# westi024/RadTxfr

Measured on AMD Instinct MI355X. Metric: wavenumber*layer points/s (32-layer TUD, 500-6000 cm^-1 @ 0.001 cm^-1), higher is better.
Workload: dtype f32; 1 GPU; C3: 32-layer TUD (tau,Lu,Ld) StandardAtmosphere rows 1-32, 500-6000 cm^-1 @ 0.001 cm^-1; n_wavenumbers=5500000, n_layers=32, n_lines=100000, n_angles=30, line_table=synthetic HITRAN-format H2O+CO2, seed 20261005, parallelism=wavenumber-sharded x1, pipelines_per_gpu=3

## Files before the change

### include/radtxfr_hip.h

```cpp
#ifndef RADTXFR_HIP_H
#define RADTXFR_HIP_H

#include <stdint.h>

#ifdef __cplusplus
extern "C" {
#endif

#define RTX_VERSION 100

typedef struct rtx_grid {
  double xmin;
  double xmax;
  double step;
  int64_t n_total;
  int64_t offset;
  int64_t n;
} rtx_grid;

int rtx_version(void);
const char* rtx_last_error(void);
int rtx_device_info(char* name_h, int len, int* n_cu_h);

typedef struct rtx_lines rtx_lines;
// ... 33 lines not shown
                         const double* T_h, const double* T_win_h, const double* p_atm_h, const double* qratio_h,
                         const double* weight_h, const double* mass_h, double dil_air, double dil_self,
                         double omega_wing, double omega_wing_hw, double intensity_threshold, double scale,
                         int profile, void* stream);

int rtx_line_prep_axis(rtx_prep* prep, const rtx_lines* lines, const double* X_h, int64_t nx, int n_layers,
                       const double* T_h, const double* p_atm_h, const double* qratio_h, const double* weight_h,
                       const double* mass_h, double dil_air, double dil_self, double omega_wing, double omega_wing_hw,
                       double intensity_threshold, double scale, int profile, void* stream);

#define RTX_MAX_DILUENTS 8
int rtx_line_prep_mix(rtx_prep* prep, const rtx_lines* lines, const rtx_grid* grid, int n_layers, const double* T_h,
                      const double* p_atm_h, const double* qratio_h, const double* weight_h, const double* mass_h,
                      int n_dil, const int32_t* dil_h, const double* frac_h, double omega_wing, double omega_wing_hw,
                      double intensity_threshold, double scale, int profile, void* stream);
int rtx_line_prep_axis_mix(rtx_prep* prep, const rtx_lines* lines, const double* X_h, int64_t nx, int n_layers,
                           const double* T_h, const double* p_atm_h, const double* qratio_h, const double* weight_h,
                           const double* mass_h, int n_dil, const int32_t* dil_h, const double* frac_h, double omega_wing,
                           double omega_wing_hw, double intensity_threshold, double scale, int profile, void* stream);

int rtx_voigt_tile_points(void);
int rtx_voigt_sum(const rtx_prep* prep, const rtx_grid* grid, int n_layers, float* out_f32,
                  double* out_f64, int64_t ld, void* stream);
int rtx_voigt_sum_axis(const rtx_prep* prep, int n_layers, float* out_f32, double* out_f64, int64_t ld, void* stream);

int rtx_line_prep_dt(rtx_prep* prep, const rtx_lines* lines, const rtx_grid* grid, int n_layers, const double* T_h,
                     const double* p_atm_h, const double* qratio_h, const double* weight_h, const double* mass_h,
                     const double* dlnsw_h, double dil_air, double dil_self, double omega_wing, double omega_wing_hw,
                     double intensity_threshold, double scale, void* stream);
int rtx_voigt_sum_dt(const rtx_prep* prep, const rtx_grid* grid, int n_layers, float* out_f32, double* out_f64,
                     int64_t ld, void* stream);

int rtx_planck(const rtx_grid* grid, const double* X, int64_t nx, const double* T, int64_t nT,
               int wavelength, double* out, void* stream);

int rtx_brightness_temperature(const double* X, int64_t nx, const double* L, int64_t m,
                               int wavelength, double bad_value, double* T_out, void* stream);
int rtx_bt2l(const double* X, int64_t nx, const double* T, int64_t m, int wavelength,
             double bad_value, double* L_out, void* stream);

int rtx_tud(const float* OD, int64_t ld, const rtx_grid* grid, int n_layers, const double* T_h,
            int n_alt, const uint8_t* mask_h, int n_mu, const double* mu_h, int n_down,
            int n_angle, int return_od, float* tau, float* Lu, float* Ld, float* Ld_angles,
            int64_t ld_out, void* stream);
#define RTX_TUD_OD_NONNEG 1u
int rtx_tud_opts(const float* OD, int64_t ld, const rtx_grid* grid, int n_layers, const double* T_h,
// ... 210 lines not shown
```

### radtxfr_amd/_lib.py

```python
import ctypes as C
import os

_HERE = os.path.dirname(os.path.abspath(__file__))
LIB_PATH = os.environ.get("RADTXFR_LIB") or os.path.join(_HERE, "libradtxfr_hip.so")


class RtxGrid(C.Structure):
    _fields_ = [("xmin", C.c_double), ("xmax", C.c_double), ("step", C.c_double),
                ("n_total", C.c_int64), ("offset", C.c_int64), ("n", C.c_int64)]


_vp, _i64, _i32, _dbl = C.c_void_p, C.c_int64, C.c_int, C.c_double
_pd = C.POINTER(C.c_double)
_gp = C.POINTER(RtxGrid)

PROTOTYPES = {
    "rtx_version": (_i32, []),
    "rtx_last_error": (C.c_char_p, []),
    "rtx_device_info": (_i32, [C.c_char_p, _i32, C.POINTER(_i32)]),
    "rtx_lines_create": (_i32, [_i64, _i32] + [_vp] * 10 + [_vp, C.POINTER(_vp)]),
    "rtx_lines_free": (_i32, [_vp]),
    "rtx_lines_count": (_i64, [_vp]),
    "rtx_prep_create": (_i32, [_vp, _i32, _i64, C.POINTER(_vp)]),
    "rtx_prep_free": (_i32, [_vp]),
    "rtx_line_prep": (_i32, [_vp, _vp, _gp, _i32, _vp, _vp, _vp, _vp, _vp, _dbl, _dbl, _dbl, _dbl, _dbl, _dbl, _vp]),
    "rtx_line_prep_profile": (_i32, [_vp, _vp, _gp, _i32, _vp, _vp, _vp, _vp, _vp, _dbl, _dbl, _dbl, _dbl, _dbl, _dbl, _i32, _vp]),
    "rtx_prep_split_bound": (_i64, [_vp]),
    "rtx_line_prep_window": (_i32, [_vp, _vp, _gp, _i32, _vp, _vp, _vp, _vp, _vp, _vp, _dbl, _dbl, _dbl, _dbl, _dbl, _dbl, _i32, _vp]),
    "rtx_line_prep_axis": (_i32, [_vp, _vp, _vp, _i64, _i32, _vp, _vp, _vp, _vp, _vp, _dbl, _dbl, _dbl, _dbl, _dbl, _dbl, _i32, _vp]),
    "rtx_voigt_sum": (_i32, [_vp, _gp, _i32, _vp, _vp, _i64, _vp]),
    "rtx_voigt_sum_axis": (_i32, [_vp, _i32, _vp, _vp, _i64, _vp]),
    "rtx_sdvoigt_sum": (_i32, [_vp, _gp, _i32, _vp, _vp, _i64, _vp]),
    "rtx_lines_set_sd": (_i32, [_vp, _vp, _vp]),
    "rtx_lines_set_deltap_self": (_i32, [_vp, _vp]),
    "rtx_lines_set_broadeners": (_i32, [_vp, _i32, _vp, _vp, _vp, _vp, _vp]),
    "rtx_line_prep_mix": (_i32, [_vp, _vp, _gp, _i32, _vp, _vp, _vp, _vp, _vp, _i32, _vp, _vp, _dbl, _dbl, _dbl, _dbl, _i32, _vp]),
    "rtx_line_prep_axis_mix": (_i32, [_vp, _vp, _vp, _i64, _i32, _vp, _vp, _vp, _vp, _vp, _i32, _vp, _vp, _dbl, _dbl, _dbl, _dbl,
                                       _i32, _vp]),
    "rtx_voigt_tile_points": (_i32, []),
    "rtx_planck": (_i32, [_gp, _vp, _i64, _vp, _i64, _i32, _vp, _vp]),
    "rtx_tud": (_i32, [_vp, _i64, _gp, _i32, _vp, _i32, _vp, _i32, _vp, _i32, _i32, _i32, _vp, _vp, _vp, _vp, _i64, _vp]),
    "rtx_tud_opts": (_i32, [_vp, _i64, _gp, _i32, _vp, _i32, _vp, _i32, _vp, _i32, _i32, _i32, _vp, _vp, _vp, _vp, _i64, _vp, C.c_uint]),
    "rtx_tud_jacobian": (_i32, [_vp, _vp, _vp, _i64, _dbl, _vp, _i32, _vp, _i64, _gp, _i32, _vp, _i32, _vp, _dbl, _i32, _i32,
                                 _i32, _vp, _i32, _i32, _vp, _i64, _vp]),
    "rtx_tud_vjp": (_i32, [_vp, _vp, _vp, _i64, _dbl, _vp, _i32, _vp, _i64, _gp, _i32, _vp, _i32, _vp, _dbl, _i32, _i32,
                            _i32, _vp, _i32, _i32, _vp, _vp, _vp, _i64, _i32, _vp, _vp]),
    "rtx_tud_vjp_max_vectors": (_i32, []),
    "rtx_line_prep_dt": (_i32, [_vp, _vp, _gp, _i32, _vp, _vp, _vp, _vp, _vp, _vp, _dbl, _dbl, _dbl, _dbl, _dbl, _dbl, _vp]),
    "rtx_voigt_sum_dt": (_i32, [_vp, _gp, _i32, _vp, _vp, _i64, _vp]),
    "rtx_tud_jacobian_dod": (_i32, [_vp, _vp, _i64, _vp, _i32, _vp, _i64, _gp, _i32, _vp, _i32, _vp, _dbl, _i32, _i32,
                                     _i32, _vp, _i32, _i32, _vp, _i64, _vp]),
    "rtx_tud_vjp_dod": (_i32, [_vp, _vp, _i64, _vp, _i32, _vp, _i64, _gp, _i32, _vp, _i32, _vp, _dbl, _i32, _i32,
                                _i32, _vp, _i32, _i32, _vp, _vp, _vp, _i64, _i32, _vp, _vp]),
# ... 113 lines not shown
```

### radtxfr_amd/csrc/rtx_voigt.hip

```cpp
#include <stdlib.h>
#include <string.h>

#include "rtx_common.h"

#include "rtx_voigt_math.h"

struct RangeArgs {
  const int* ic;
  const int* maxhw;
  const int2* win;
  long long n_lines;
  int n_tiles, tile, n_layers, n_steps;
  long long n;
  int2* ranges;
  SplitItem* items;
  int* n_items;
  long long items_cap;
};

#define RNG_G 16
__device__ __forceinline__ unsigned group_bits(unsigned long long b, int lane) { return (unsigned)(b >> (lane & 48)) & 0xffffu; }

template <bool STRICT>
__device__ __forceinline__ void bound_step(const int* __restrict__ ic, int& lo, int& hi, int v, int sub, int lane) {
// ... 124 lines not shown
    if (out_f32) RTX_HIP(hipMemset2DAsync(out_f32, ld * sizeof(float), 0, grid->n * sizeof(float), n_layers, st));
    if (out_f64) RTX_HIP(hipMemset2DAsync(out_f64, ld * sizeof(double), 0, grid->n * sizeof(double), n_layers, st));
    return 0;
  }
  return rtx_voigt_sum_scatter(P, grid, n_layers, out_f32, out_f64, ld, st, launch_tile_ranges, voigt_kernel_choice() == 0);
}

bool rtx_voigt_layers_ok(const rtx_prep* P) {
  return P && !P->axis && P->n_lines > 0 && voigt_kernel_choice() == 0 && !(P->split_bound > 0 && P->items.get());
}
int rtx_voigt_sum_layers(const rtx_prep* P, const rtx_grid* grid, int n_layers, float* out_f32, int64_t ld, void* stream,
                         const VoigtLayers& sel) {
  if (!rtx_voigt_layers_ok(P)) RTX_FAIL("internal: a layer subset on a prologue that cannot take one");
  if (rtx_check_grid(grid)) return 1;
  if (n_layers < 1 || n_layers != P->n_layers) RTX_FAIL("n_layers=%d does not match the last rtx_line_prep (%d)", n_layers, P->n_layers);
  if (!out_f32) RTX_FAIL("the output is NULL");
  if (ld < grid->n) RTX_FAIL("ld=%lld < n=%lld", (long long)ld, (long long)grid->n);
  if (sel.n_a < 0 || sel.n_y < sel.n_a || sel.n_y < 1 || sel.k_a < 0 || sel.k_a + sel.n_a > n_layers || sel.k_b < 0 ||
      sel.k_b + (sel.n_y - sel.n_a) > n_layers)
    RTX_FAIL("internal: layer subset outside [0,%d)", n_layers);
  if (grid->n == 0) return 0;
  return rtx_voigt_sum_scatter(P, grid, n_layers, out_f32, nullptr, ld, (hipStream_t)stream, launch_tile_ranges, 1, &sel);
}
```

### radtxfr_amd/csrc/rtx_voigt_scatter.hip

```cpp
#include "rtx_common.h"

#include "rtx_voigt_math.h"

#include "cheb8_64.inc"
#include "cheb16_tile.inc"
#include <vector>

#ifndef RTX_SC_ABLATE
#define RTX_SC_ABLATE 0
#endif
#ifndef RTX_SC_ASYM
#define RTX_SC_ASYM 1
#endif
#ifndef RTX_SC_OUTER
#define RTX_SC_OUTER 1
#endif
#ifndef RTX_SC_ROWS
#define RTX_SC_ROWS 16
#endif
#ifndef RTX_SC_NEAR
#define RTX_SC_NEAR 2
#endif
static_assert(RTX_SC_ROWS <= 31, "row masks are 32-bit");

// ... 300 lines not shown
#endif
#ifndef SC_EDGE_LIST
#define SC_EDGE_LIST 1
#endif
#ifndef SC_EDGE_CAP
#define SC_EDGE_CAP 32
#endif
#ifndef SC_EDGE_UNROLL
#define SC_EDGE_UNROLL 2
#endif
#ifndef RTX_SC_TILE_LEVEL
#define RTX_SC_TILE_LEVEL 1
#endif
#define RTX_SC_TILE_DIST 512
#ifndef RTX_SC_RED_REG
#define RTX_SC_RED_REG 1
#endif
#ifndef RTX_SC_MERGE
#define RTX_SC_MERGE 1
#endif
#ifndef RTX_SC_BAND_SPLIT
#define RTX_SC_BAND_SPLIT 1
#endif
#ifndef SC_ENT_CAP
#define SC_ENT_CAP (SC_EDGE_LIST ? 16 : 32)
#endif
template <bool SMALLY, bool PARTS = false>
__device__ __forceinline__ void nodal_tile(const ScArgs& a, const int b_or_tile, const int k, const int2 part_rng = make_int2(0, 0),
                                           float* __restrict__ part_out = nullptr, const unsigned done_rows = 0u) {
  constexpr int ROWS = RTX_SC_ROWS;
  constexpr int TILE = 64 * ROWS;
  __shared__ float s_acc[SC_NW][TILE];
  __shared__ float4 s_ent[SC_NW][SC_ENT_CAP][4];
  __shared__ float4 s_edge[SC_NW][SC_EDGE_LIST ? SC_EDGE_CAP : 1][2];
  __shared__ float s_nodsum[RTX_SC_ROWS][CHEB_N];
  static_assert((RTX_SC_ROWS * CHEB_N + TCHEB_N + 1) * 4 <= SC_ENT_CAP * 64, "row sums + tile sums fit in one wave's entry list");

  const int tile = part_out ? b_or_tile : xcd_tile(b_or_tile);
  if (tile >= a.n_tiles) return;
  const int wave = __builtin_amdgcn_readfirstlane((int)(threadIdx.x >> 6));
  const int lane = threadIdx.x & 63;
  const long long n = a.g.n;
  const int ia = tile * TILE;
  const int ib = (int)((long long)ia + TILE < n ? (long long)ia + TILE : n);
  const int nt = ib - ia;
  const LineRec* __restrict__ rec = a.rec + (size_t)k * (size_t)a.n_lines;
  const LineRec64* __restrict__ rec64 = a.rec64 + (size_t)k * (size_t)a.n_lines;
  const int2 rng = part_out ? part_rng : a.ranges[(size_t)k * a.n_tiles + tile];
  float* __restrict__ acc = s_acc[wave];
#pragma unroll
  for (int r = 0; r < ROWS; ++r) acc[r * 64 + lane] = 0.f;
  const float lanef = (float)lane;
  bool touched = false;
// ... 1 lines not shown
  long long t_prev = RTX_SC_STAMP ? (long long)clock64() : 0;
  const long long t_begin = t_prev;

  const int l = lane >> 3, j = lane & 7;
  float nod[ROWS];
#pragma unroll
  for (int r = 0; r < ROWS; ++r) nod[r] = 0.f;
  constexpr bool TILE_LEVEL = RTX_SC_TILE_LEVEL && ROWS == 16;
#ifndef RTX_SC_OFF_LDS
#define RTX_SC_OFF_LDS 0
#endif
#if !RTX_SC_OFF_LDS
  const float off_j = CHEB_OFF[j];
#endif
  if (lane < 8) {
    int lt = lane;
    if (SMALLY) asm volatile("" : "+v"(lt));
    s_nodsum[wave][lane] = CHEB_OFF[lt];
    if (TILE_LEVEL) s_nodsum[SC_NW + wave][lane] = TCHEB_OFF[lt];
  }
  float tnod_a = 0.f, tnod_b = 0.f;
  int n_tile_members = 0;
  int n_ent = 0;
  float4(*__restrict__ ent)[4] = s_ent[wave];
  auto below = [](unsigned long long m) -> int {
    return (int)__builtin_amdgcn_mbcnt_hi((unsigned)(m >> 32), __builtin_amdgcn_mbcnt_lo((unsigned)m, 0u));
  };
  auto pull = [](int src_lane, float v) -> float {
    return __int_as_float(__builtin_amdgcn_ds_bpermute(src_lane << 2, __float_as_int(v)));
  };

  static_assert(ROWS <= 16, "an entry packs its row masks as 16-bit halves");
  auto drain = [&]() {
    for (int e = 0; e < n_ent; ++e) {
      const float4 e0 = ent[e][0], e1 = ent[e][1], e2 = ent[e][2], e3 = ent[e][3];
      LineRec q;
      q.a = e0.x; q.c = e0.y; q.b1 = e0.z; q.b0 = e0.w;
      q.Ay = e1.x; q.Ay0 = e1.y; q.y = e1.z; q.A = e1.w;
      const float u0 = e2.x + lanef, ulo = e2.y, uhi = e2.z, zw_f = e2.w;
      const unsigned w0 = (unsigned)__builtin_amdgcn_readfirstlane(__float_as_int(e3.x));
      const unsigned w1 = (unsigned)__builtin_amdgcn_readfirstlane(__float_as_int(e3.y));
      unsigned m_pp = w0 & 0xffffu, m_ed = w0 >> 16, m_bd = w1 & 0xffffu, m_cut = w1 >> 16;
      if (!PARTS) {
        m_pp &= ~done_rows; m_ed &= ~done_rows;
      }
      auto slot = [&]() -> int { return __builtin_amdgcn_readfirstlane(__float_as_int(ent[e][3].z)); };
      STAMP(3);
      if (RTX_SC_ABLATE & 4) m_pp = m_ed = 0u;
      while (m_pp) {
        const int r = __builtin_ctz(m_pp);
        m_pp &= m_pp - 1u;
        float* p = acc + r * 64 + lane;
        float x0, n0, d0;
        farwing(u0 + (float)(64 * r), q, x0, n0, d0);
        p[0] = fmaf(n0, d0, p[0]);
      }
      while (m_ed) {
        const int r = __builtin_ctz(m_ed);
        m_ed &= m_ed - 1u;
        float* p = acc + r * 64 + lane;
        const float u = u0 + (float)(64 * r);
        float x0, n0, d0;
        farwing(u, q, x0, n0, d0);
        n0 = (u >= ulo && u < uhi) ? n0 : 0.f;
        p[0] = fmaf(n0, d0, p[0]);
      }
// ... 15 lines not shown
              p[0] = fmaf(num, rden, p[0]);
            }
          } else {
            for (; r < r_end; ++r) {
              float* p = acc + r * 64 + lane;
              float num, rden;
              band_row<0, false, 0>(a, rec64, slot, q, u0 + (float)(64 * r), ia + 64 * r + lane, zw_f, ulo, uhi, false, num, rden, touched);
              p[0] = fmaf(num, rden, p[0]);
            }
          }
        }
        while (m_cut) {
          const int r = __builtin_ctz(m_cut);
          m_cut &= m_cut - 1u;
          float* p = acc + r * 64 + lane;
          float num, rden;
          band_row<SMALLY ? 2 : 0>(a, rec64, slot, q, u0 + (float)(64 * r), ia + 64 * r + lane, zw_f, ulo, uhi, small_y, num, rden, touched);
          p[0] = fmaf(num, rden, p[0]);
        }
      }
      STAMP(5);
    }
    n_ent = 0;
  };

  int n_edge = 0;
  float4(*__restrict__ edg)[2] = s_edge[wave];
  auto edge_one = [&](const float4& E0, const float4& E1, int pk) {
    const int r = (pk >> 7) & 31, t = pk & 127;
    const bool right = (pk >> 12) & 1;
    float* p = acc + r * 64 + lane;
    const float u = E1.z + lanef;
    const float x = fmaf(u, E0.x, E0.y);
    const float xx = x * x;
    float num = fmaf(xx, E1.x, E1.y);
    const float rden = __builtin_amdgcn_rcpf(fmaf(xx + E0.z, xx, E0.w));
    const bool inside = (lane >= t) != right;
    num = inside ? num : 0.f;
    p[0] = fmaf(num, rden, p[0]);
  };
  auto drain_edges = [&]() {
    for (int e = 0; e < n_edge; e += SC_EDGE_UNROLL) {
      float4 E0[SC_EDGE_UNROLL], E1[SC_EDGE_UNROLL];
      int pk[SC_EDGE_UNROLL];
#pragma unroll
      for (int q = 0; q < SC_EDGE_UNROLL; ++q) {
        const int eq = e + q < n_edge ? e + q : e;
        E0[q] = edg[eq][0];
        E1[q] = edg[eq][1];
      }
#pragma unroll
      for (int q = 0; q < SC_EDGE_UNROLL; ++q) pk[q] = __builtin_amdgcn_readfirstlane(__float_as_int(E1[q].w));
#pragma unroll
      for (int q = 0; q < SC_EDGE_UNROLL; ++q)
        if (e + q < n_edge) edge_one(E0[q], E1[q], pk[q]);
    }
    n_edge = 0;
  };

  for (int base = rng.x + wave; base < rng.y; base += 64 * SC_NW) {
    const int slot = base + SC_NW * lane;
    const bool valid = slot < rng.y;
    const float4* __restrict__ pr = reinterpret_cast<const float4*>(rec + (valid ? slot : rng.y - 1));
    const float4 f0 = pr[0];
    const float4 f1 = pr[1];
    const float4 f2 = pr[2];
    const int qi0 = __float_as_int(f2.x), qlo = __float_as_int(f2.y), qhi = __float_as_int(f2.z), qzw = __float_as_int(f2.w);
    const bool reach = valid && qhi > ia && qlo < ib;
    const RowGeom g = row_geom(qi0, qlo, qhi, qzw, ia, nt);
    auto bits = [](int lo, int hi) -> unsigned {
      return hi > lo ? (((1u << hi) - 1u) & ~((1u << lo) - 1u)) : 0u;
    };
    const unsigned m_reach = reach ? bits(g.r_lo, g.r_hi) : 0u;
    const unsigned m_in = reach ? bits(g.c0, g.c1) : 0u;
    const unsigned m_near = bits(g.n0 > 0 ? g.n0 : 0, (g.n1 < ROWS - 1 ? g.n1 : ROWS - 1) + 1);
    const unsigned m_band = bits(g.z0, g.z1 + 1);
    const unsigned m_far = (RTX_SC_ABLATE & 2) ? 0u : (m_in & ~m_near);
    const unsigned m_bd = m_reach & m_band;
    const unsigned m_pp = m_in & m_near & ~m_band;
    const unsigned m_ed = (RTX_SC_ABLATE & 16) ? 0u : (m_reach & ~m_in & ~m_band);
    const float ub = (float)(ia - qi0);
    constexpr unsigned ALL_ROWS = (1u << ROWS) - 1u;
    if (RTX_SC_STAMP && __ballot(m_pp == 0xffffffffu)) t_ph[7] += 1;
    STAMP(0);

    bool edge_only = false;
    if (SC_EDGE_LIST) {
      const bool single = m_pp == 0u && m_bd == 0u && m_ed != 0u && (m_ed & (m_ed - 1u)) == 0u;
      const int re = single ? __builtin_ctz(m_ed) : 0;
      const bool left = g.part_l && re == g.r_lo, rightc = g.part_r && re == g.r_hi - 1;
      edge_only = single && (left != rightc) && !(RTX_SC_ABLATE & 8);
      const int dlo = qlo - ia, dhi = qhi - ia;
      const int t = left ? dlo - 64 * re : dhi - 64 * re;
      const int pk = (t & 127) | (re << 7) | (left ? 0 : 1 << 12);
      bool emit = edge_only;
      unsigned long long eb = __ballot(emit);
      while (eb) {
        const int room = SC_EDGE_CAP - n_edge;
        const int r = below(eb);
        if (emit && r < room) {
          float4* d = edg[n_edge + r];
          d[0] = f0;
          d[1] = make_float4(f1.x, f1.y, ub + (float)(64 * re), __int_as_float(pk));
          emit = false;
        }
        const int cnt = __popcll(eb);
        n_edge += cnt < room ? cnt : room;
        if (n_edge == SC_EDGE_CAP) drain_edges();
        eb = __ballot(emit);
      }
    }
    {
      const unsigned m_cut = f1.z < 1.0f ? m_bd : m_bd & ~m_in;
      const unsigned w0 = m_pp | (m_ed << 16), w1 = m_bd | (m_cut << 16);
      bool emit = !(RTX_SC_ABLATE & 8) && !edge_only && (w0 | w1) != 0u;
      unsigned long long eb = __ballot(emit);
      while (eb) {
        const int room = SC_ENT_CAP - n_ent;
        const int r = below(eb);
        if (emit && r < room) {
          float4* d = ent[n_ent + r];
          d[0] = f0;
          d[1] = f1;
          d[2] = make_float4(ub, (float)(qlo - qi0), (float)(qhi - qi0), qzw > 0 ? (float)qzw : -1.0f);
          d[3] = make_float4(__int_as_float((int)w0), __int_as_float((int)w1), __int_as_float(slot), __int_as_float((f1.z < 1.0f ? 1 : 0) | (f1.z >= 6.0f ? 2 : 0)));
          emit = false;
        }
        const int cnt = __popcll(eb);
        n_ent += cnt < room ? cnt : room;
        if (n_ent == SC_ENT_CAP) drain();
        eb = __ballot(emit);
      }
    }
    STAMP(1);
    bool is_t = false;
    if (TILE_LEVEL) {
      is_t = m_far == ALL_ROWS && (ia - qi0 >= RTX_SC_TILE_DIST || qi0 - (ia + TILE - 1) >= RTX_SC_TILE_DIST);
      const unsigned long long tb = __ballot(is_t);
      if (tb) {
        const int nT = __popcll(tb);
        n_tile_members += nT;
        const float toff_a = s_nodsum[SC_NW + wave][j];
        const int src = __builtin_amdgcn_ds_permute((is_t ? below(tb) : 63) << 2, lane);
        for (int g0 = 0; g0 < nT; g0 += 8) {
          const int e = g0 + l;
          const int sl = __builtin_amdgcn_ds_bpermute(e << 2, src);
          const float qa = pull(sl, f0.x), qc = pull(sl, f0.y), qb1 = pull(sl, f0.z), qb0 = pull(sl, f0.w);
          float qAy = pull(sl, f1.x), qAy0 = pull(sl, f1.y);
          const float qub = pull(sl, ub);
          if (e >= nT) { qAy = 0.f; qAy0 = 0.f; }
          const float xa = fmaf(qub, qa, fmaf(toff_a, qa, qc));
          const float xb = fmaf(qub, qa, fmaf(1023.0f - toff_a, qa, qc));
// ... 8 lines not shown
      const int nF = __popcll(__ballot(m_far == ALL_ROWS && !is_t)), nP = __popcll(__ballot(m_far != 0u && m_far != ALL_ROWS));
      merged = ((nF + nP + 7) >> 3) < ((nF + 7) >> 3) + ((nP + 7) >> 3);
    }
#pragma unroll
    for (int pass = 0; pass < 2; ++pass) {
      const bool is_m = pass == 0 ? (m_far == ALL_ROWS && !is_t && !merged) : (m_far != 0u && (m_far != ALL_ROWS || (merged && !is_t)));
      const unsigned long long rb = __ballot(is_m);
      if (!rb) continue;
      const int nR = __popcll(rb);
#if RTX_SC_OFF_LDS
      const float off_j = s_nodsum[wave][j];
#endif
      const int src = __builtin_amdgcn_ds_permute((is_m ? below(rb) : 63) << 2, lane);
      for (int g0 = 0; g0 < nR; g0 += 8) {
        const int e = g0 + l;
        const int sl = __builtin_amdgcn_ds_bpermute(e << 2, src);
        const float qa = pull(sl, f0.x), qc = pull(sl, f0.y), qb1 = pull(sl, f0.z), qb0 = pull(sl, f0.w);
        float qAy = pull(sl, f1.x), qAy0 = pull(sl, f1.y);
        const float qub = pull(sl, ub);
        const float x0 = fmaf(qub, qa, fmaf(off_j, qa, qc));
        const float dx = 64.0f * qa;
        if (pass == 0) {
          if (e >= nR) { qAy = 0.f; qAy0 = 0.f; }
#pragma unroll
          for (int r = 0; r < ROWS; ++r) {
            const float x = fmaf((float)r, dx, x0);
            const float xx = x * x;
            const float num = fmaf(xx, qAy, qAy0);
            const float rden = __builtin_amdgcn_rcpf(fmaf(xx + qb1, xx, qb0));
            nod[r] = fmaf(num, rden, nod[r]);
          }
        } else {
          int mf = __builtin_amdgcn_ds_bpermute(sl << 2, (int)m_far);
          mf = e < nR ? mf : 0;
#define SC_PART_ROW(r_)                                                                  \
          if (r_ < ROWS) {                                                                 \
            const float x = fmaf((float)(r_), dx, x0);                                     \
            const float xx = x * x;                                                        \
            float num = fmaf(xx, qAy, qAy0);                                               \
            const float rden = __builtin_amdgcn_rcpf(fmaf(xx + qb1, xx, qb0));             \
            int mb;                                                                        \
            asm("v_bfe_i32 %0, %1, %2, 1" : "=v"(mb) : "v"(mf), "n"(r_));                  \
            num = __int_as_float(__float_as_int(num) & mb);                                \
            nod[r_ < ROWS ? r_ : 0] = fmaf(num, rden, nod[r_ < ROWS ? r_ : 0]);            \
          }
          SC_PART_ROW(0) SC_PART_ROW(1) SC_PART_ROW(2) SC_PART_ROW(3) SC_PART_ROW(4) SC_PART_ROW(5) SC_PART_ROW(6) SC_PART_ROW(7)
          SC_PART_ROW(8) SC_PART_ROW(9) SC_PART_ROW(10) SC_PART_ROW(11) SC_PART_ROW(12) SC_PART_ROW(13) SC_PART_ROW(14) SC_PART_ROW(15)
          SC_PART_ROW(16) SC_PART_ROW(17) SC_PART_ROW(18) SC_PART_ROW(19) SC_PART_ROW(20) SC_PART_ROW(21) SC_PART_ROW(22) SC_PART_ROW(23)
          SC_PART_ROW(24) SC_PART_ROW(25) SC_PART_ROW(26) SC_PART_ROW(27) SC_PART_ROW(28) SC_PART_ROW(29) SC_PART_ROW(30)
#undef SC_PART_ROW
        }
      }
    }
    STAMP(2);
  }
  drain();
  if (SC_EDGE_LIST) drain_edges();

  const int ln = (int)__builtin_amdgcn_mbcnt_hi(~0u, __builtin_amdgcn_mbcnt_lo(~0u, 0u));
#if RTX_SC_RED_REG
  auto ror8 = [](float v) -> float {
    return v + __int_as_float(__builtin_amdgcn_update_dpp(0, __float_as_int(v), 0x128, 0xf, 0xf, true));
  };
  auto swap16 = [](float a, float b) -> float {
    const auto s = __builtin_amdgcn_permlane16_swap((unsigned)__float_as_int(a), (unsigned)__float_as_int(b), false, false);
    return __int_as_float((int)s[0]) + __int_as_float((int)s[1]);
  };
  auto swap32 = [](float a, float b) -> float {
    const auto s = __builtin_amdgcn_permlane32_swap((unsigned)__float_as_int(a), (unsigned)__float_as_int(b), false, false);
    return __int_as_float((int)s[0]) + __int_as_float((int)s[1]);
// ... 16 lines not shown
#pragma unroll
  for (int r = 0; r < ROWS; ++r) {
    float v = nod[r];
    v += __shfl_xor(v, 8);
    v += __shfl_xor(v, 16);
    v += __shfl_xor(v, 32);
    if (lane < 8) reinterpret_cast<float*>(&s_ent[wave][0][0])[r * CHEB_N + lane] = v;
  }
  if (TILE_LEVEL) {
    float va = tnod_a, vb = tnod_b;
    va += __shfl_xor(va, 8);  vb += __shfl_xor(vb, 8);
    va += __shfl_xor(va, 16); vb += __shfl_xor(vb, 16);
    va += __shfl_xor(va, 32); vb += __shfl_xor(vb, 32);
    float* ts = reinterpret_cast<float*>(&s_ent[wave][0][0]) + ROWS * CHEB_N;
    if (lane < 8) { ts[lane] = va; ts[15 - lane] = vb; }
    if (lane == 0) ts[16] = __int_as_float(n_tile_members);
  }
#endif
  STAMP(2);
  __syncthreads();
  STAMP(6);
  static_assert(SC_NW == 1 || SC_NW == 2 || SC_NW == 4, "one, two or four waves per workgroup");
  for (int o = wave * 64 + ln; o < ROWS * CHEB_N; o += 64 * SC_NW) {
    float v = reinterpret_cast<const float*>(&s_ent[0][0][0])[o];
    if constexpr (SC_NW >= 2) v += reinterpret_cast<const float*>(&s_ent[1][0][0])[o];
    if constexpr (SC_NW == 4) v += reinterpret_cast<const float*>(&s_ent[2][0][0])[o] + reinterpret_cast<const float*>(&s_ent[3][0][0])[o];
    if (TILE_LEVEL) {
      int any = 0;
#pragma unroll
      for (int w = 0; w < SC_NW; ++w) any |= __float_as_int(reinterpret_cast<const float*>(&s_ent[w][0][0])[ROWS * CHEB_N + 16]);
      if (any) {
        float c = 0.f;
#pragma unroll
        for (int t = 0; t < TCHEB_N; ++t) {
          float tsum = reinterpret_cast<const float*>(&s_ent[0][0][0])[ROWS * CHEB_N + t];
          if constexpr (SC_NW >= 2) tsum += reinterpret_cast<const float*>(&s_ent[1][0][0])[ROWS * CHEB_N + t];
          if constexpr (SC_NW == 4)
            tsum += reinterpret_cast<const float*>(&s_ent[2][0][0])[ROWS * CHEB_N + t] + reinterpret_cast<const float*>(&s_ent[3][0][0])[ROWS * CHEB_N + t];
          c = fmaf(TCHEB_M[t][o], tsum, c);
        }
        v += c;
      }
    }
    s_nodsum[o >> 3][o & 7] = v;
  }
  __syncthreads();
// ... 14 lines not shown
      if constexpr (SC_NW == 4) pp += s_acc[2][t] + s_acc[3][t];
      const float v = pp + f;
      if (part_out) {
        part_out[t] = v;
      } else if (i < (long long)ib) {
        const size_t o = (size_t)k * (size_t)a.ld + (size_t)i;
        if (a.out32) a.out32[o] = v;
        if (a.out64) a.out64[o] = (double)v * a.inv_scale;
      }
    }
  }
  if (RTX_SC_STAMP && !part_out) {
    t_ph[7] = (long long)clock64() - t_begin;
    if (lane == 0) {
      unsigned long long* o = a.stamp + ((size_t)(blockIdx.y * gridDim.x + blockIdx.x) * SC_NW + wave) * SC_NSTAMP;
      for (int i = 0; i < SC_NSTAMP; ++i) o[i] = (unsigned long long)t_ph[i];
    }
  }
}

#ifndef RTX_SC_WAVES_SMALLY
#define RTX_SC_WAVES_SMALLY 4
#endif
template <bool SMALLY>
__global__ __launch_bounds__(64 * SC_NW, SMALLY ? RTX_SC_WAVES_SMALLY : RTX_SC_WAVES) void voigt_nodal_kernel(ScArgs a) {
  const int k = sc_layer(a, blockIdx.y);
  if ((a.smally[k] != 0) != SMALLY) return;
  if (SMALLY) {
    for (int b = blockIdx.x; b < 8 * a.tiles_per_xcd; b += gridDim.x) {
      const unsigned done_rows = sc_done_rows(a, b);
      if (done_rows == 0xFFFFu) continue;
      nodal_tile<true>(a, b, k, make_int2(0, 0), nullptr, done_rows);
      __syncthreads();
    }
  } else {
    const unsigned done_rows = sc_done_rows(a, blockIdx.x);
    if (done_rows == 0xFFFFu) return;
    nodal_tile<false>(a, blockIdx.x, k, make_int2(0, 0), nullptr, done_rows);
  }
}

template <bool SMALLY>
__global__ __launch_bounds__(64 * SC_NW, SMALLY ? RTX_SC_WAVES_SMALLY : RTX_SC_WAVES) void voigt_nodal_parts_kernel(ScArgs a) {
  const int i = blockIdx.x;
  if (i >= *a.n_items) return;
  const SplitItem it = a.items[i];
  if ((a.smally[it.k] != 0) != SMALLY) return;
  nodal_tile<SMALLY, true>(a, it.tile, it.k, make_int2(it.lo, it.hi), a.part_ws + (size_t)i * (size_t)(64 * RTX_SC_ROWS));
}

__global__ __launch_bounds__(256) void split_combine_kernel(ScArgs a) {
  constexpr int TILE = 64 * RTX_SC_ROWS;
  const int i = blockIdx.x;
  if (i >= *a.n_items) return;
  const SplitItem it = a.items[i];
  if (it.part != 1) return;
  const long long ia = (long long)it.tile * TILE;
  for (int t = threadIdx.x; t < TILE; t += 256) {
    const long long p = ia + t;
    if (p >= a.g.n) break;
    const size_t o = (size_t)it.k * (size_t)a.ld + (size_t)p;
// ... 28 lines not shown
  ScArgs a;
  a.rec = P->rec.get(); a.rec64 = P->rec64.get(); a.ranges = P->ranges.get(); a.smally = P->smally; a.n_lines = P->n_lines;
  a.n_tiles = n_tiles; a.tiles_per_xcd = xcd_slots(n_tiles);
  a.g = to_dev(grid);
  a.out32 = out_f32; a.out64 = out_f64; a.ld = ld; a.inv_scale = 1.0 / P->scale;
  a.stamp = nullptr;
  a.items = P->items.get(); a.n_items = P->n_items; a.part_ws = P->part_ws.get();
  a.n_a = sel ? sel->n_a : n_layers; a.k_a = sel ? sel->k_a : 0; a.k_b = sel ? sel->k_b : 0; a.done = sel ? sel->done : nullptr;
#if RTX_SC_STAMP
  static unsigned long long* d_stamp = nullptr;
  static size_t stamp_cap = 0;
  const size_t n_stamp = (size_t)8 * a.tiles_per_xcd * n_layers * SC_NW * SC_NSTAMP;
  if (stamp_cap < n_stamp) {
    if (d_stamp) RTX_HIP(hipFree(d_stamp));
    RTX_HIP(hipMalloc(&d_stamp, n_stamp * sizeof(unsigned long long)));
    stamp_cap = n_stamp;
  }
  RTX_HIP(hipMemsetAsync(d_stamp, 0, n_stamp * sizeof(unsigned long long), st));
  a.stamp = d_stamp;
#endif
  static int lds_pad = -1;
  if (lds_pad < 0) { const char* e = getenv("RADTXFR_DEBUG_LDS_PAD"); lds_pad = e ? atoi(e) : 0; }
  if (nodal) {
    hipLaunchKernelGGL((voigt_nodal_kernel<false>), dim3(8 * a.tiles_per_xcd, n_y), dim3(64 * SC_NW), (size_t)lds_pad, st, a);
    RTX_LAUNCH_CHECK();
    hipLaunchKernelGGL((voigt_nodal_kernel<true>), dim3(8 * ((a.tiles_per_xcd + 15) / 16), n_y), dim3(64 * SC_NW), 0, st, a);
    if (P->split_bound > 0 && P->items.get()) {
      RTX_LAUNCH_CHECK();
      const unsigned cap = (unsigned)P->split_bound;
      hipLaunchKernelGGL((voigt_nodal_parts_kernel<false>), dim3(cap), dim3(64 * SC_NW), 0, st, a);
      hipLaunchKernelGGL((voigt_nodal_parts_kernel<true>), dim3(cap), dim3(64 * SC_NW), 0, st, a);
      hipLaunchKernelGGL(split_combine_kernel, dim3(cap), dim3(256), 0, st, a);
    }
  } else {
    hipLaunchKernelGGL((voigt_scatter_kernel<false>), dim3(8 * a.tiles_per_xcd, n_layers), dim3(256), 0, st, a);
  }
  RTX_LAUNCH_CHECK();
#if RTX_SC_STAMP
  {
    std::vector<unsigned long long> hbuf(n_stamp);
    RTX_HIP(hipMemcpyAsync(hbuf.data(), d_stamp, n_stamp * sizeof(unsigned long long), hipMemcpyDeviceToHost, st));
    RTX_HIP(hipStreamSynchronize(st));
    if (const char* fn = getenv("RADTXFR_STAMP_FILE")) {
      FILE* fh = fopen(fn, "wb");
      if (fh) { fwrite(hbuf.data(), sizeof(unsigned long long), n_stamp, fh); fclose(fh); }
    }
    double h[SC_NSTAMP] = {0};
// ... 13 lines not shown
```

### radtxfr_amd/engine.py

```python
import ctypes as C
from typing import NamedTuple, Optional

import numpy as np
import torch

from . import _lib, tips

TUD_MAX_MU = 8
TUD_OD_NONNEG = 1
CTUD_OD_SCRATCH = 1

CBOLTS = 1.380648813e-16
TREF = 296.0


def volumeConcentration(p, T):
    return (p / 9.869233e-7) / (CBOLTS * T)


class trace_range:
    enabled = bool(int(__import__("os").environ.get("RADTXFR_ROCTX", "0") or 0))

    def __init__(self, name):
        self.name = name
# ... 391 lines not shown

def _check_outputs(nL, ld, out_f32, out_f64):
    for o, dt in ((out_f32, torch.float32), (out_f64, torch.float64)):
        if o is not None:
            assert o.dtype == dt and o.is_cuda and o.is_contiguous() and o.shape == (nL, ld), (o.dtype, o.shape)


def voigt_sum(lines, grid, T, p_atm, weight, out_f32=None, out_f64=None, dil_air=1.0, dil_self=0.0, omega_wing=0.0,
              omega_wing_hw=50.0, intensity_threshold=0.0, scale=1.0, partitionFunction=None, qratio=None, mass=None,
              profile=0, diluent=None):
    lib = _lib.load()
    nL, env = _prologue_inputs(lines, T, p_atm, weight, partitionFunction, qratio, mass)
    plan = lines.plan(nL, grid.n)
    st = _stream_ptr()
    _line_prep(lib.rtx_line_prep_profile, lib.rtx_line_prep_mix, (plan._h, lines._h, grid.byref(), nL, *(e[1] for e in env)),
               lines, nL, diluent, dil_air, dil_self, omega_wing, omega_wing_hw, intensity_threshold, scale, profile, st)
    ld = grid.n
    _check_outputs(nL, ld, out_f32, out_f64)
    if int(profile) == 3:
        _lib.check(lib.rtx_sdvoigt_sum(plan._h, grid.byref(), nL, _ptr(out_f32), _ptr(out_f64), ld, st))
    else:
        _lib.check(lib.rtx_voigt_sum(plan._h, grid.byref(), nL, _ptr(out_f32), _ptr(out_f64), ld, st))
    return out_f32, out_f64


def voigt_sum_axis(lines, X, T, p_atm, weight, out_f32=None, out_f64=None, dil_air=1.0, dil_self=0.0, omega_wing=0.0,
                   omega_wing_hw=50.0, intensity_threshold=0.0, scale=1.0, partitionFunction=None, qratio=None, mass=None,
                   profile=0, diluent=None):
    lib = _lib.load()
    X = _host_axis("voigt_sum_axis", X)
    if int(profile) not in (0, 1, 2):
        raise NotImplementedError("voigt_sum_axis: profile %d; an explicit axis takes Voigt (0), Lorentz (1) or Doppler (2)"
                                  % int(profile))
    nL, env = _prologue_inputs(lines, T, p_atm, weight, partitionFunction, qratio, mass)
    nx = X.size
    plan = lines.plan(nL, max(nx, 1))
    st = _stream_ptr()
    _line_prep(lib.rtx_line_prep_axis, lib.rtx_line_prep_axis_mix,
               (plan._h, lines._h, X.ctypes.data_as(C.c_void_p), nx, nL, *(e[1] for e in env)),
               lines, nL, diluent, dil_air, dil_self, omega_wing, omega_wing_hw, intensity_threshold, scale, profile, st)
    _check_outputs(nL, nx, out_f32, out_f64)
    _lib.check(lib.rtx_voigt_sum_axis(plan._h, nL, _ptr(out_f32), _ptr(out_f64), nx, st))
    return out_f32, out_f64


class HtPlan:
# ... 1197 lines not shown
```

Baseline: 127.2 billion wavenumber*layer points/s.

## Skip done rows in nodal Voigt tiles via row-subset sum entry point

Adds rtx_voigt_sum_rows, which sums a layer range and accepts a per-tile skip-rows mask. It also adds a HIDE instantiation of the fp32 nodal tile kernel that leaves finished (opaque) row groups out of the nodal evaluation, out of the stored entry and edge lists, and out of the final writeback. The aim is to avoid Voigt work on spectral rows whose output is no longer needed. In exchange it adds extra ballots and counters in the emit loops, plus a second kernel instantiation. The non-HIDE path now ignores done_rows entirely, which changes behaviour when a.done is unset.

```diff
diff --git a/include/radtxfr_hip.h b/include/radtxfr_hip.h
--- a/include/radtxfr_hip.h
+++ b/include/radtxfr_hip.h
@@ -79,6 +79,8 @@
 int rtx_voigt_tile_points(void);
 int rtx_voigt_sum(const rtx_prep* prep, const rtx_grid* grid, int n_layers, float* out_f32,
                   double* out_f64, int64_t ld, void* stream);
+int rtx_voigt_sum_rows(const rtx_prep* prep, const rtx_grid* grid, int n_layers, float* out_f32, int64_t ld, int k_lo,
+                       int k_hi, const unsigned char* skip_rows, void* stream, unsigned flags);
 int rtx_voigt_sum_axis(const rtx_prep* prep, int n_layers, float* out_f32, double* out_f64, int64_t ld, void* stream);
 
 int rtx_line_prep_dt(rtx_prep* prep, const rtx_lines* lines, const rtx_grid* grid, int n_layers, const double* T_h,
diff --git a/radtxfr_amd/_lib.py b/radtxfr_amd/_lib.py
--- a/radtxfr_amd/_lib.py
+++ b/radtxfr_amd/_lib.py
@@ -29,6 +29,7 @@
     "rtx_line_prep_window": (_i32, [_vp, _vp, _gp, _i32, _vp, _vp, _vp, _vp, _vp, _vp, _dbl, _dbl, _dbl, _dbl, _dbl, _dbl, _i32, _vp]),
     "rtx_line_prep_axis": (_i32, [_vp, _vp, _vp, _i64, _i32, _vp, _vp, _vp, _vp, _vp, _dbl, _dbl, _dbl, _dbl, _dbl, _dbl, _i32, _vp]),
     "rtx_voigt_sum": (_i32, [_vp, _gp, _i32, _vp, _vp, _i64, _vp]),
+    "rtx_voigt_sum_rows": (_i32, [_vp, _gp, _i32, _vp, _i64, _i32, _i32, _vp, _vp, C.c_uint]),
     "rtx_voigt_sum_axis": (_i32, [_vp, _i32, _vp, _vp, _i64, _vp]),
     "rtx_sdvoigt_sum": (_i32, [_vp, _gp, _i32, _vp, _vp, _i64, _vp]),
     "rtx_lines_set_sd": (_i32, [_vp, _vp, _vp]),
diff --git a/radtxfr_amd/csrc/rtx_voigt.hip b/radtxfr_amd/csrc/rtx_voigt.hip
--- a/radtxfr_amd/csrc/rtx_voigt.hip
+++ b/radtxfr_amd/csrc/rtx_voigt.hip
@@ -170,3 +170,27 @@
   if (grid->n == 0) return 0;
   return rtx_voigt_sum_scatter(P, grid, n_layers, out_f32, nullptr, ld, (hipStream_t)stream, launch_tile_ranges, 1, &sel);
 }
+
+extern "C" int rtx_voigt_sum_rows(const rtx_prep* P, const rtx_grid* grid, int n_layers, float* out_f32, int64_t ld, int k_lo,
+                                  int k_hi, const unsigned char* skip_rows, void* stream, unsigned flags) {
+  if (flags != 0) RTX_FAIL("rtx_voigt_sum_rows: flags=%u, none is defined", flags);
+  if (!P) RTX_FAIL("prep is NULL");
+  if (P->axis) RTX_FAIL("rtx_voigt_sum_rows: the last prologue was rtx_line_prep_axis, whose sum takes no subset");
+  if (voigt_kernel_choice() != 0) RTX_FAIL("rtx_voigt_sum_rows: RADTXFR_VOIGT_KERNEL=scatter, the point-by-point kernel takes no subset");
+  if (P->split_bound > 0 && P->items.get())
+    RTX_FAIL("rtx_voigt_sum_rows: the table has a hot-tile bound (%lld extra parts), whose tiles take no subset", (long long)P->split_bound);
+  if (n_layers < 1 || n_layers != P->n_layers) RTX_FAIL("n_layers=%d does not match the last rtx_line_prep (%d)", n_layers, P->n_layers);
+  if (k_lo < 0 || k_hi < k_lo || k_hi > n_layers) RTX_FAIL("rtx_voigt_sum_rows: layers [%d,%d) outside [0,%d)", k_lo, k_hi, n_layers);
+  if ((uintptr_t)skip_rows & 15u) RTX_FAIL("rtx_voigt_sum_rows: skip_rows is not 16-byte aligned");
+  if (rtx_check_grid(grid)) return 1;
+  if (!out_f32) RTX_FAIL("the output is NULL");
+  if (ld < grid->n) RTX_FAIL("ld=%lld < n=%lld", (long long)ld, (long long)grid->n);
+  if (k_lo == k_hi || grid->n == 0) return 0;
+  if (P->n_lines == 0) {
+    if (skip_rows) RTX_FAIL("rtx_voigt_sum_rows: skip_rows on a table without lines");
+    RTX_HIP(hipMemset2DAsync(out_f32 + (size_t)k_lo * (size_t)ld, ld * sizeof(float), 0, grid->n * sizeof(float), k_hi - k_lo, (hipStream_t)stream));
+    return 0;
+  }
+  const VoigtLayers sel{k_hi - k_lo, k_lo, 0, k_hi - k_lo, skip_rows, true};
+  return rtx_voigt_sum_layers(P, grid, n_layers, out_f32, ld, stream, sel);
+}
diff --git a/radtxfr_amd/csrc/rtx_voigt_scatter.hip b/radtxfr_amd/csrc/rtx_voigt_scatter.hip
--- a/radtxfr_amd/csrc/rtx_voigt_scatter.hip
+++ b/radtxfr_amd/csrc/rtx_voigt_scatter.hip
@@ -346,13 +346,26 @@
 #ifndef RTX_SC_BAND_SPLIT
 #define RTX_SC_BAND_SPLIT 1
 #endif
+#ifndef RTX_SC_HIDE_ROWS
+#define RTX_SC_HIDE_ROWS 4
+#endif
+#ifndef RTX_SC_HIDE_LISTS
+#define RTX_SC_HIDE_LISTS 1
+#endif
 #ifndef SC_ENT_CAP
 #define SC_ENT_CAP (SC_EDGE_LIST ? 16 : 32)
 #endif
-template <bool SMALLY, bool PARTS = false>
+template <bool SMALLY, bool PARTS = false, bool HIDE = false>
 __device__ __forceinline__ void nodal_tile(const ScArgs& a, const int b_or_tile, const int k, const int2 part_rng = make_int2(0, 0),
                                            float* __restrict__ part_out = nullptr, const unsigned done_rows = 0u) {
+  static_assert(!HIDE || (!SMALLY && !PARTS), "done rows are left out by the fp32 tile kernel alone");
   constexpr int ROWS = RTX_SC_ROWS;
+  constexpr int HIDE_G = HIDE ? RTX_SC_HIDE_ROWS : 0;
+  constexpr bool HIDE_L = HIDE && RTX_SC_HIDE_LISTS != 0;
+  auto grp_done = [&](int r0) -> bool {
+    constexpr unsigned G = (1u << (HIDE_G > 0 ? HIDE_G : 1)) - 1u;
+    return HIDE_G > 0 && ((done_rows >> r0) & G) == G;
+  };
   constexpr int TILE = 64 * ROWS;
   __shared__ float s_acc[SC_NW][TILE];
   __shared__ float4 s_ent[SC_NW][SC_ENT_CAP][4];
@@ -400,6 +413,7 @@
   float tnod_a = 0.f, tnod_b = 0.f;
   int n_tile_members = 0;
   int n_ent = 0;
+  int n_ent_w = 0;
   float4(*__restrict__ ent)[4] = s_ent[wave];
   auto below = [](unsigned long long m) -> int {
     return (int)__builtin_amdgcn_mbcnt_hi((unsigned)(m >> 32), __builtin_amdgcn_mbcnt_lo((unsigned)m, 0u));
@@ -410,7 +424,8 @@
 
   static_assert(ROWS <= 16, "an entry packs its row masks as 16-bit halves");
   auto drain = [&]() {
-    for (int e = 0; e < n_ent; ++e) {
+    const int n_stored = HIDE_L ? n_ent_w : n_ent;
+    for (int e = 0; e < n_stored; ++e) {
       const float4 e0 = ent[e][0], e1 = ent[e][1], e2 = ent[e][2], e3 = ent[e][3];
       LineRec q;
       q.a = e0.x; q.c = e0.y; q.b1 = e0.z; q.b0 = e0.w;
@@ -419,7 +434,7 @@
       const unsigned w0 = (unsigned)__builtin_amdgcn_readfirstlane(__float_as_int(e3.x));
       const unsigned w1 = (unsigned)__builtin_amdgcn_readfirstlane(__float_as_int(e3.y));
       unsigned m_pp = w0 & 0xffffu, m_ed = w0 >> 16, m_bd = w1 & 0xffffu, m_cut = w1 >> 16;
-      if (!PARTS) {
+      if (!PARTS && !HIDE_L) {
         m_pp &= ~done_rows; m_ed &= ~done_rows;
       }
       auto slot = [&]() -> int { return __builtin_amdgcn_readfirstlane(__float_as_int(ent[e][3].z)); };
@@ -481,9 +496,11 @@
       STAMP(5);
     }
     n_ent = 0;
+    n_ent_w = 0;
   };
 
   int n_edge = 0;
+  int n_edge_w = 0;
   float4(*__restrict__ edg)[2] = s_edge[wave];
   auto edge_one = [&](const float4& E0, const float4& E1, int pk) {
     const int r = (pk >> 7) & 31, t = pk & 127;
@@ -499,12 +516,13 @@
     p[0] = fmaf(num, rden, p[0]);
   };
   auto drain_edges = [&]() {
-    for (int e = 0; e < n_edge; e += SC_EDGE_UNROLL) {
+    const int n_stored = HIDE_L ? n_edge_w : n_edge;
+    for (int e = 0; e < n_stored; e += SC_EDGE_UNROLL) {
       float4 E0[SC_EDGE_UNROLL], E1[SC_EDGE_UNROLL];
       int pk[SC_EDGE_UNROLL];
 #pragma unroll
       for (int q = 0; q < SC_EDGE_UNROLL; ++q) {
-        const int eq = e + q < n_edge ? e + q : e;
+        const int eq = e + q < n_stored ? e + q : e;
         E0[q] = edg[eq][0];
         E1[q] = edg[eq][1];
       }
@@ -512,9 +530,10 @@
       for (int q = 0; q < SC_EDGE_UNROLL; ++q) pk[q] = __builtin_amdgcn_readfirstlane(__float_as_int(E1[q].w));
 #pragma unroll
       for (int q = 0; q < SC_EDGE_UNROLL; ++q)
-        if (e + q < n_edge) edge_one(E0[q], E1[q], pk[q]);
+        if (e + q < n_stored) edge_one(E0[q], E1[q], pk[q]);
     }
     n_edge = 0;
+    n_edge_w = 0;
   };
 
   for (int base = rng.x + wave; base < rng.y; base += 64 * SC_NW) {
@@ -553,40 +572,54 @@
       const int t = left ? dlo - 64 * re : dhi - 64 * re;
       const int pk = (t & 127) | (re << 7) | (left ? 0 : 1 << 12);
       bool emit = edge_only;
+      const bool live = !HIDE_L || !((done_rows >> re) & 1u);
       unsigned long long eb = __ballot(emit);
       while (eb) {
         const int room = SC_EDGE_CAP - n_edge;
         const int r = below(eb);
-        if (emit && r < room) {
-          float4* d = edg[n_edge + r];
+        const bool take = emit && r < room;
+        const unsigned long long lb = HIDE_L ? __ballot(take && live) : 0ull;
+        if (take && live) {
+          float4* d = edg[HIDE_L ? n_edge_w + below(lb) : n_edge + r];
           d[0] = f0;
           d[1] = make_float4(f1.x, f1.y, ub + (float)(64 * re), __int_as_float(pk));
-          emit = false;
         }
+        emit = emit && !take;
         const int cnt = __popcll(eb);
         n_edge += cnt < room ? cnt : room;
+        if (HIDE_L) n_edge_w += __popcll(lb);
         if (n_edge == SC_EDGE_CAP) drain_edges();
         eb = __ballot(emit);
       }
     }
     {
-      const unsigned m_cut = f1.z < 1.0f ? m_bd : m_bd & ~m_in;
-      const unsigned w0 = m_pp | (m_ed << 16), w1 = m_bd | (m_cut << 16);
-      bool emit = !(RTX_SC_ABLATE & 8) && !edge_only && (w0 | w1) != 0u;
+      unsigned l_bd = m_bd;
+      if (HIDE_L) {
+        const unsigned lv = m_bd & ~done_rows;
+        l_bd = lv ? bits(__builtin_ctz(lv), 32 - __builtin_clz(lv)) : 0u;
+      }
+      const unsigned l_pp = HIDE_L ? m_pp & ~done_rows : m_pp, l_ed = HIDE_L ? m_ed & ~done_rows : m_ed;
+      const unsigned m_cut = f1.z < 1.0f ? l_bd : l_bd & ~m_in;
+      const unsigned w0 = l_pp | (l_ed << 16), w1 = l_bd | (m_cut << 16);
+      bool emit = !(RTX_SC_ABLATE & 8) && !edge_only && (m_pp | m_ed | m_bd) != 0u;
+      const bool live = !HIDE_L || (w0 | w1) != 0u;
       unsigned long long eb = __ballot(emit);
       while (eb) {
         const int room = SC_ENT_CAP - n_ent;
         const int r = below(eb);
-        if (emit && r < room) {
-          float4* d = ent[n_ent + r];
+        const bool take = emit && r < room;
+        const unsigned long long lb = HIDE_L ? __ballot(take && live) : 0ull;
+        if (take && live) {
+          float4* d = ent[HIDE_L ? n_ent_w + below(lb) : n_ent + r];
           d[0] = f0;
           d[1] = f1;
           d[2] = make_float4(ub, (float)(qlo - qi0), (float)(qhi - qi0), qzw > 0 ? (float)qzw : -1.0f);
           d[3] = make_float4(__int_as_float((int)w0), __int_as_float((int)w1), __int_as_float(slot), __int_as_float((f1.z < 1.0f ? 1 : 0) | (f1.z >= 6.0f ? 2 : 0)));
-          emit = false;
         }
+        emit = emit && !take;
         const int cnt = __popcll(eb);
         n_ent += cnt < room ? cnt : room;
+        if (HIDE_L) n_ent_w += __popcll(lb);
         if (n_ent == SC_ENT_CAP) drain();
         eb = __ballot(emit);
       }
@@ -641,13 +674,19 @@
         const float dx = 64.0f * qa;
         if (pass == 0) {
           if (e >= nR) { qAy = 0.f; qAy0 = 0.f; }
-#pragma unroll
-          for (int r = 0; r < ROWS; ++r) {
-            const float x = fmaf((float)r, dx, x0);
-            const float xx = x * x;
-            const float num = fmaf(xx, qAy, qAy0);
-            const float rden = __builtin_amdgcn_rcpf(fmaf(xx + qb1, xx, qb0));
-            nod[r] = fmaf(num, rden, nod[r]);
+          constexpr int RG = HIDE_G > 0 ? HIDE_G : ROWS;
+          static_assert(ROWS % RG == 0, "row groups tile the rows");
+#pragma unroll
+          for (int r0 = 0; r0 < ROWS; r0 += RG) {
+            if (grp_done(r0)) continue;
+#pragma unroll
+            for (int r = r0; r < r0 + RG; ++r) {
+              const float x = fmaf((float)r, dx, x0);
+              const float xx = x * x;
+              const float num = fmaf(xx, qAy, qAy0);
+              const float rden = __builtin_amdgcn_rcpf(fmaf(xx + qb1, xx, qb0));
+              nod[r] = fmaf(num, rden, nod[r]);
+            }
           }
         } else {
           int mf = __builtin_amdgcn_ds_bpermute(sl << 2, (int)m_far);
@@ -663,8 +702,14 @@
             num = __int_as_float(__float_as_int(num) & mb);                                \
             nod[r_ < ROWS ? r_ : 0] = fmaf(num, rden, nod[r_ < ROWS ? r_ : 0]);            \
           }
-          SC_PART_ROW(0) SC_PART_ROW(1) SC_PART_ROW(2) SC_PART_ROW(3) SC_PART_ROW(4) SC_PART_ROW(5) SC_PART_ROW(6) SC_PART_ROW(7)
-          SC_PART_ROW(8) SC_PART_ROW(9) SC_PART_ROW(10) SC_PART_ROW(11) SC_PART_ROW(12) SC_PART_ROW(13) SC_PART_ROW(14) SC_PART_ROW(15)
+          static_assert(HIDE_G == 0 || HIDE_G == 1 || HIDE_G == 2 || HIDE_G == 4, "rows per done-row test");
+#define SC_PART_ONE(r_) if (HIDE_G != 1 || !grp_done(r_)) { SC_PART_ROW(r_) }
+#define SC_PART_TWO(r_) if (HIDE_G != 2 || !grp_done(r_)) { SC_PART_ONE(r_) SC_PART_ONE(r_ + 1) }
+#define SC_PART_FOUR(r_) if (HIDE_G != 4 || !grp_done(r_)) { SC_PART_TWO(r_) SC_PART_TWO(r_ + 2) }
+          SC_PART_FOUR(0) SC_PART_FOUR(4) SC_PART_FOUR(8) SC_PART_FOUR(12)
+#undef SC_PART_FOUR
+#undef SC_PART_TWO
+#undef SC_PART_ONE
           SC_PART_ROW(16) SC_PART_ROW(17) SC_PART_ROW(18) SC_PART_ROW(19) SC_PART_ROW(20) SC_PART_ROW(21) SC_PART_ROW(22) SC_PART_ROW(23)
           SC_PART_ROW(24) SC_PART_ROW(25) SC_PART_ROW(26) SC_PART_ROW(27) SC_PART_ROW(28) SC_PART_ROW(29) SC_PART_ROW(30)
 #undef SC_PART_ROW
@@ -727,6 +772,7 @@
   STAMP(6);
   static_assert(SC_NW == 1 || SC_NW == 2 || SC_NW == 4, "one, two or four waves per workgroup");
   for (int o = wave * 64 + ln; o < ROWS * CHEB_N; o += 64 * SC_NW) {
+    if (HIDE && ((done_rows >> (o >> 3)) & 1u)) continue;
     float v = reinterpret_cast<const float*>(&s_ent[0][0][0])[o];
     if constexpr (SC_NW >= 2) v += reinterpret_cast<const float*>(&s_ent[1][0][0])[o];
     if constexpr (SC_NW == 4) v += reinterpret_cast<const float*>(&s_ent[2][0][0])[o] + reinterpret_cast<const float*>(&s_ent[3][0][0])[o];
@@ -787,8 +833,9 @@
 #ifndef RTX_SC_WAVES_SMALLY
 #define RTX_SC_WAVES_SMALLY 4
 #endif
-template <bool SMALLY>
+template <bool SMALLY, bool HIDE = false>
 __global__ __launch_bounds__(64 * SC_NW, SMALLY ? RTX_SC_WAVES_SMALLY : RTX_SC_WAVES) void voigt_nodal_kernel(ScArgs a) {
+  static_assert(!(SMALLY && HIDE), "the fp64 instantiation treats done rows as before");
   const int k = sc_layer(a, blockIdx.y);
   if ((a.smally[k] != 0) != SMALLY) return;
   if (SMALLY) {
@@ -798,10 +845,12 @@
       nodal_tile<true>(a, b, k, make_int2(0, 0), nullptr, done_rows);
       __syncthreads();
     }
-  } else {
+  } else if (HIDE) {
     const unsigned done_rows = sc_done_rows(a, blockIdx.x);
     if (done_rows == 0xFFFFu) return;
-    nodal_tile<false>(a, blockIdx.x, k, make_int2(0, 0), nullptr, done_rows);
+    nodal_tile<false, false, true>(a, blockIdx.x, k, make_int2(0, 0), nullptr, done_rows);
+  } else {
+    nodal_tile<false>(a, blockIdx.x, k);
   }
 }
 
@@ -876,7 +925,8 @@
   static int lds_pad = -1;
   if (lds_pad < 0) { const char* e = getenv("RADTXFR_DEBUG_LDS_PAD"); lds_pad = e ? atoi(e) : 0; }
   if (nodal) {
-    hipLaunchKernelGGL((voigt_nodal_kernel<false>), dim3(8 * a.tiles_per_xcd, n_y), dim3(64 * SC_NW), (size_t)lds_pad, st, a);
+    if (a.done) hipLaunchKernelGGL((voigt_nodal_kernel<false, true>), dim3(8 * a.tiles_per_xcd, n_y), dim3(64 * SC_NW), (size_t)lds_pad, st, a);
+    else hipLaunchKernelGGL((voigt_nodal_kernel<false>), dim3(8 * a.tiles_per_xcd, n_y), dim3(64 * SC_NW), (size_t)lds_pad, st, a);
     RTX_LAUNCH_CHECK();
     hipLaunchKernelGGL((voigt_nodal_kernel<true>), dim3(8 * ((a.tiles_per_xcd + 15) / 16), n_y), dim3(64 * SC_NW), 0, st, a);
     if (P->split_bound > 0 && P->items.get()) {
diff --git a/radtxfr_amd/engine.py b/radtxfr_amd/engine.py
--- a/radtxfr_amd/engine.py
+++ b/radtxfr_amd/engine.py
@@ -437,6 +437,21 @@
     else:
         _lib.check(lib.rtx_voigt_sum(plan._h, grid.byref(), nL, _ptr(out_f32), _ptr(out_f64), ld, st))
     return out_f32, out_f64
+
+
+def voigt_sum_rows(lines, grid, n_layers, out_f32, k_lo=0, k_hi=None, skip_rows=None):
+    lib = _lib.load()
+    nL = int(n_layers)
+    k_hi = nL if k_hi is None else int(k_hi)
+    _check_outputs(nL, grid.n, out_f32, None)
+    if skip_rows is not None:
+        tile = lib.rtx_voigt_tile_points()
+        need = -(-grid.n // tile) * (tile // 64)
+        assert skip_rows.dtype == torch.uint8 and skip_rows.is_cuda and skip_rows.is_contiguous() and skip_rows.numel() >= need, \
+            (skip_rows.dtype, skip_rows.shape, need)
+    _lib.check(lib.rtx_voigt_sum_rows(lines.plan(nL, grid.n)._h, grid.byref(), nL, _ptr(out_f32), grid.n, int(k_lo), k_hi,
+                                      _ptr(skip_rows), _stream_ptr(), 0))
+    return out_f32
 
 
 def voigt_sum_axis(lines, X, T, p_atm, weight, out_f32=None, out_f64=None, dil_air=1.0, dil_self=0.0, omega_wing=0.0,
```

New measurement: 137.4 billion wavenumber*layer points/s (median of 6 runs). +8.0%, better.
